# goofoo/SLR

Hardware: AMD Instinct MI355X
Metric: Msamples/sec @1024spp 1280x720 (unidirectional path tracing, Cornell_Box_Spheres-shaped scene) (higher is better)
Workload: dtype f32; 1 GPU; BASELINE configs[1]: Cornell_Box_Spheres walls/light/camera (TestScenes/Cornell_Box_Spheres.txt:8-107,132-138) + two tessellated spheres (aluminium mirror, Lambert), 4428 triangles, RGB mode, 1280x720, 1024 spp, seed 1509761209; stripes=0, tree=host binned SAH

## Files before the change

### include/slrhip.h

```cpp
#ifndef SLRHIP_H
#define SLRHIP_H

#include <stddef.h>
#include <stdint.h>

#ifdef __cplusplus
extern "C" {
#endif

#define SLRHIP_VERSION 7

enum {
    SLRHIP_OK = 0,
    SLRHIP_ERR_INVALID_ARGUMENT = 1,
    SLRHIP_ERR_NO_DEVICE = 2,
    SLRHIP_ERR_HIP = 3,
    SLRHIP_ERR_NO_SCENE = 4,
    SLRHIP_ERR_UNSUPPORTED = 5,
    SLRHIP_ERR_OUT_OF_MEMORY = 6
};

enum {
    SLRHIP_MODE_RGB = 0,
    SLRHIP_MODE_SPECTRAL = 1
// ... 146 lines not shown
    uint64_t shadow_rays;
    uint64_t iterations;
    uint64_t bvh_nodes;
    uint64_t bvh_depth;
    double   build_seconds;
    uint64_t bvh_leaf_references;
} slrhip_counters;

enum {
    SLRHIP_KERNEL_TRACE = 0,
    SLRHIP_KERNEL_SHADE = 1,
    SLRHIP_KERNEL_TAIL = 2,
    SLRHIP_KERNEL_COUNT = 3
};
typedef struct slrhip_profile {
    uint64_t launches[SLRHIP_KERNEL_COUNT];
    double   milliseconds[SLRHIP_KERNEL_COUNT];
    uint64_t rays[2];
    uint64_t nodes[2];
    uint64_t triangles[2];
    uint64_t slot_visits;
} slrhip_profile;

#define SLRHIP_FLAG_DYNAMIC_INSTANCED 1024u
#define SLRHIP_FLAG_DYNAMIC_GEOMETRY 512u
#define SLRHIP_FLAG_NO_PRIMARY_PASS 256u
#define SLRHIP_FLAG_TAIL_KERNEL 128u
#define SLRHIP_FLAG_BVH_SPATIAL_SPLITS 64u
#define SLRHIP_FLAG_BVH_DEVICE_BUILD 4u
#define SLRHIP_FLAG_TEST_DEVICE_ERROR 16u
#define SLRHIP_FLAG_TIME_KERNELS   1u
#define SLRHIP_FLAG_COUNT_TRAVERSAL 2u

typedef struct slrhip_ctx slrhip_ctx;

int slrhip_create(const slrhip_config* config, slrhip_ctx** out_ctx);
int slrhip_destroy(slrhip_ctx* ctx);

int slrhip_upload_scene(slrhip_ctx* ctx, const slrhip_scene_desc* scene);

int slrhip_render_begin(slrhip_ctx* ctx, const slrhip_render_settings* settings, slrhip_shard shard);

int slrhip_render(slrhip_ctx* ctx, uint32_t spp_begin, uint32_t spp_count, void* stream);

int slrhip_resolve_framebuffer(slrhip_ctx* ctx, float* device_dst, size_t num_floats, void* stream);

// ... 308 lines not shown
```

### include/slrhip_debug.h

```cpp
#ifndef SLRHIP_DEBUG_H
#define SLRHIP_DEBUG_H

#include "slrhip.h"

#ifdef __cplusplus
extern "C" {
#endif

int slrhip_bsdf_queries(slrhip_ctx* ctx, uint32_t material, uint32_t n, const float* queries,
                        float wl_offset, float u_lambda, float* out);

int slrhip_debug_work_distribution(uint32_t num_pixels, uint32_t num_slots, uint32_t num_passes, uint32_t run_length,
                                   uint32_t* counts, uint32_t* queue_lengths);

int slrhip_debug_render_plan(int32_t width, int32_t height, uint32_t shard_index, uint32_t shard_count, uint32_t stripes, int32_t mode,
                             uint32_t num_passes, uint64_t budget_bytes, uint32_t* plan, uint32_t* windows, uint32_t max_windows,
                             uint32_t* num_windows, uint32_t* pixels, uint32_t max_pixels);

int slrhip_debug_primary_plan(uint32_t num_pixels, uint32_t num_passes, uint32_t config_flags, int32_t scene_class, uint32_t* plan);

int slrhip_debug_primary_samples(slrhip_ctx* ctx, uint64_t* samples);

int slrhip_debug_primary_entries(uint32_t num_pixels, uint32_t first_pass, uint32_t num_passes, uint32_t window_passes, uint64_t* entries);

int slrhip_debug_primary_stream_plan(uint32_t num_pixels, uint32_t num_passes, uint32_t config_flags, int32_t scene_class, uint64_t* entries);

int slrhip_debug_primary_stream_entries(slrhip_ctx* ctx, uint64_t* entries);

int slrhip_debug_camera_draws(int32_t device, uint32_t n, const uint32_t* tuples, uint32_t* out);

int slrhip_debug_adaptive_blocks(uint32_t spp_min, uint32_t spp_step, uint32_t spp_max, uint32_t* blocks, uint32_t max_blocks,
                                 uint32_t* num_blocks);

int slrhip_debug_modulate_check(const slrhip_modulate_desc* desc);

int slrhip_debug_reproject_check(const slrhip_reproject_desc* desc);

int slrhip_debug_motion_check(int32_t have_render, uint32_t num_instances, const slrhip_motion_desc* desc, uint32_t spp_begin, uint32_t spp_count);

int slrhip_debug_motion_vertices_check(int32_t have_render, uint32_t num_instances, uint32_t config_flags, uint32_t tree_builder,
                                       const slrhip_motion_vertices_desc* desc, uint32_t spp_begin, uint32_t spp_count);

int slrhip_debug_environment_check(const slrhip_environment_desc* desc);

int slrhip_debug_environment(slrhip_ctx* ctx, uint32_t what, float* host_dst, size_t num_floats);

int slrhip_debug_instance_update_check(int32_t have_scene, uint32_t num_instances, const void* device_src, uint32_t first_instance,
                                       uint32_t count);

int slrhip_debug_top_level(slrhip_ctx* ctx, uint32_t what, void* host_dst, size_t num_words);
// ... 43 lines not shown
```

### slr_amd/abi.py

```python
import ctypes as C
import os

import numpy as np

ROOT = os.path.dirname(os.path.dirname(os.path.abspath(__file__)))

MODE_RGB, MODE_SPECTRAL = 0, 1
MAT_MATTE, MAT_METAL, MAT_GLASS, MAT_MF_METAL, MAT_MF_GLASS, MAT_WARD, MAT_ASHIKHMIN, MAT_MULTI = 0, 1, 2, 3, 4, 5, 6, 7
MULTI_INVERSE_0, MULTI_INVERSE_1 = 1, 2
SPEC_RGB_ONLY, SPEC_UPSAMPLED, SPEC_REGULAR, SPEC_IRREGULAR = 0, 1, 2, 3

vertex_dtype = np.dtype([("position", "<f4", 3), ("normal", "<f4", 3), ("tangent", "<f4", 3),
                         ("texcoord", "<f4", 2)])
triangle_dtype = np.dtype([("v", "<u4", 3), ("material", "<u4")])
material_dtype = np.dtype([("type", "<u4"), ("spectrum", "<i4", 3), ("param", "<f4"), ("emittance", "<i4"), ("param2", "<f4"), ("reserved", "<u4")])
spectrum_dtype = np.dtype([("kind", "<u4"), ("rgb", "<f4", 3), ("u", "<f4"), ("v", "<f4"), ("scale", "<f4"),
                           ("lambda_min", "<f4"), ("lambda_max", "<f4"), ("num_samples", "<u4"),
                           ("data_offset", "<u4"), ("reserved", "<u4")])


texture_dtype = np.dtype([("kind", "<u4"), ("offset", "<f4", 2), ("scale", "<f4", 2), ("spectrum", "<i4", 2), ("value", "<f4", 2),
                          ("reserved", "<u4", 3)])
instance_dtype = np.dtype([("first_triangle", "<u4"), ("num_triangles", "<u4"), ("local_to_world", "<f4", 16), ("world_to_local", "<f4", 16)])
instance_transform_dtype = np.dtype([("local_to_world", "<f4", 16), ("world_to_local", "<f4", 16)])
# ... 187 lines not shown
                ("spectra", C.c_void_p), ("num_spectra", C.c_uint32),
                ("spectrum_data", C.c_void_p), ("num_spectrum_data", C.c_uint32),
                ("textures", C.c_void_p), ("num_textures", C.c_uint32),
                ("reserved", C.c_uint32 * 2)]


DENOISE_SIGMA_DISTANCE = 0.1


def noise_metric(summary, metric=NOISE_RMSE):
    if summary["pixels"] == 0:
        return 0.0
    rmse = float(np.sqrt(np.float64(summary["sum_variance_of_mean"]) / np.float64(summary["pixels"])))
    if metric == NOISE_RMSE:
        return rmse
    mean = float(np.float64(summary["sum_mean"]) / np.float64(summary["pixels"]))
    return float("inf") if mean == 0.0 else rmse / mean


FLAG_TIME_KERNELS, FLAG_COUNT_TRAVERSAL, FLAG_BVH_DEVICE_BUILD, FLAG_TEST_DEVICE_ERROR, FLAG_BVH_SPATIAL_SPLITS, FLAG_TAIL_KERNEL = 1, 2, 4, 16, 64, 128
FLAG_NO_PRIMARY_PASS = 256
FLAG_DYNAMIC_GEOMETRY = 512
FLAG_DYNAMIC_INSTANCED = 1024
MAX_STRIPES = 64
KERNEL_NAMES = ("trace", "shade", "tail")

DEFAULT_SEED = 1509761209


class Scene:

    def __init__(self, vertices, triangles, materials, spectra, spectrum_data, camera, env=None, name="scene", textures=None,
                 texture_texels=None, texture_texels_uvs=None, instances=None):
        self.vertices = np.ascontiguousarray(vertices, dtype=vertex_dtype)
        self.triangles = np.ascontiguousarray(triangles, dtype=triangle_dtype)
        mats = np.asarray(materials)
        if mats.dtype != material_dtype:
            conv = np.zeros(len(mats), dtype=material_dtype)
            for name in mats.dtype.names:
                conv[name] = mats[name]
            mats = conv
        self.materials = np.ascontiguousarray(mats, dtype=material_dtype)
        self.spectra = np.ascontiguousarray(spectra, dtype=spectrum_dtype)
        self.spectrum_data = np.ascontiguousarray(spectrum_data, dtype=np.float32)
        self.camera = camera
        self.textures = np.ascontiguousarray(textures if textures is not None else np.zeros(0, texture_dtype), dtype=texture_dtype)
# ... 94 lines not shown
```

### slr_amd/binding.py

```python
import ctypes as C
import os
import subprocess

import numpy as np

from . import abi

CSRC = os.path.join(os.path.dirname(os.path.abspath(__file__)), "csrc")
LIB_PATH = os.path.join(CSRC, "libslrhip.so")

EXPORTS = ["slrhip_create", "slrhip_destroy", "slrhip_upload_scene", "slrhip_render_begin", "slrhip_render",
           "slrhip_resolve_framebuffer", "slrhip_reduce_framebuffer", "slrhip_read_framebuffer", "slrhip_synchronize", "slrhip_get_counters",
           "slrhip_components", "slrhip_get_profile", "slrhip_trace_rays", "slrhip_intersect_rays", "slrhip_test_visibility",
           "slrhip_query_status", "slrhip_render_features", "slrhip_resolve_features", "slrhip_read_features", "slrhip_camera_rays", "slrhip_features_status",
           "slrhip_statistics_begin", "slrhip_resolve_statistics", "slrhip_read_statistics", "slrhip_statistics_summary", "slrhip_render_until", "slrhip_sample_luminance",
           "slrhip_render_adaptive", "slrhip_resolve_framebuffer_mean", "slrhip_read_framebuffer_mean", "slrhip_adaptive_active", "slrhip_debug_adaptive_blocks",
           "slrhip_denoise", "slrhip_denoise_scratch_bytes", "slrhip_tonemap", "slrhip_tonemap_bytes",
           "slrhip_render_albedo", "slrhip_resolve_albedo", "slrhip_read_albedo", "slrhip_modulate", "slrhip_debug_modulate_check",
           "slrhip_clamp_begin", "slrhip_resolve_clamp", "slrhip_read_clamp", "slrhip_clamp_summary", "slrhip_clamp_sample", "slrhip_debug_fold",
           "slrhip_set_environment", "slrhip_env_importance", "slrhip_env_texels_to_uvs", "slrhip_debug_environment_check", "slrhip_debug_environment",
           "slrhip_set_instance_transforms", "slrhip_instances_status", "slrhip_instance_world_box", "slrhip_set_camera",
           "slrhip_debug_instance_update_check", "slrhip_debug_top_level",
           "slrhip_rebuild_top_level", "slrhip_top_level_cost", "slrhip_top_level_key", "slrhip_debug_top_level_rebuild_check",
           "slrhip_debug_top_level_plan", "slrhip_debug_top_level_reseat", "slrhip_debug_top_level_cost", "slrhip_debug_top_level_rebuild",
           "slrhip_render_motion", "slrhip_resolve_motion", "slrhip_read_motion", "slrhip_motion_camera", "slrhip_motion_sample", "slrhip_reproject",
           "slrhip_debug_motion_check", "slrhip_debug_reproject_check",
           "slrhip_render_motion_vertices", "slrhip_motion_sample_vertices", "slrhip_debug_motion_vertices_check",
           "slrhip_debug_tree", "slrhip_debug_host_tree", "slrhip_debug_quantize_nodes",
           "slrhip_set_vertices", "slrhip_geometry_status", "slrhip_debug_geometry_update_check", "slrhip_debug_geometry",
           "slrhip_debug_geometry_update_check2",
           "slrhip_set_materials", "slrhip_set_texture_texels", "slrhip_debug_materials_update_check", "slrhip_debug_materials",
           "slrhip_bsdf_queries", "slrhip_debug_work_distribution", "slrhip_debug_render_plan", "slrhip_debug_primary_plan", "slrhip_debug_primary_samples", "slrhip_debug_primary_entries", "slrhip_debug_primary_stream_entries", "slrhip_debug_primary_stream_plan", "slrhip_debug_camera_draws", "slrhip_sample_seed", "slrhip_upsample", "slrhip_resolve_upsampled", "slrhip_spectrum_to_rgb", "slrhip_tonemap_bgr8", "slrhip_save_bmp",
           "slrhip_last_error_string", "slrhip_version"]


class HipLibraryMissing(RuntimeError):
    pass


class SlrHipError(RuntimeError):
    pass


_lib = None


def build_library():
    subprocess.check_call(["make", "-s", "-C", CSRC])


def load_library():
    global _lib
    if _lib is not None:
        return _lib
    path = os.environ.get("SLRHIP_LIBRARY", LIB_PATH)
# ... 117 lines not shown
                                                                   C.c_uint32]),
                           ("slrhip_debug_geometry", [C.c_void_p, C.c_uint32, C.c_void_p, C.c_size_t])):
        if path == LIB_PATH or hasattr(lib, name):
            getattr(lib, name).argtypes = argtypes
    if path == LIB_PATH or hasattr(lib, "slrhip_debug_geometry_update_check2"):
        lib.slrhip_debug_geometry_update_check2.argtypes = [C.c_int32, C.c_int32, C.c_int32, C.c_uint32, C.c_uint32, C.c_uint32, C.c_void_p, C.c_uint32, C.c_uint32]
    for name, argtypes in (("slrhip_set_materials", [C.c_void_p, C.POINTER(abi.MaterialsDesc), C.c_void_p]),
                           ("slrhip_set_texture_texels", [C.c_void_p, C.c_uint32, C.c_void_p, C.c_uint32, C.c_void_p]),
                           ("slrhip_debug_materials_update_check", [C.c_int32, C.POINTER(abi.SceneDesc), C.c_int32, C.POINTER(abi.MaterialsDesc),
                                                                    C.c_void_p, C.c_size_t]),
                           ("slrhip_debug_materials", [C.c_void_p, C.c_uint32, C.c_void_p, C.c_size_t])):
        if path == LIB_PATH or hasattr(lib, name):
            getattr(lib, name).argtypes = argtypes
    if path == LIB_PATH or hasattr(lib, "slrhip_sample_luminance"):
        lib.slrhip_sample_luminance.restype = C.c_float
    if path == LIB_PATH or hasattr(lib, "slrhip_debug_primary_plan"):
        lib.slrhip_debug_primary_plan.argtypes = [C.c_uint32, C.c_uint32, C.c_uint32, C.c_int32, C.c_void_p]
        lib.slrhip_debug_primary_samples.argtypes = [C.c_void_p, C.POINTER(C.c_uint64)]
    if path == LIB_PATH or hasattr(lib, "slrhip_debug_camera_draws"):
        lib.slrhip_debug_primary_entries.argtypes = [C.c_uint32, C.c_uint32, C.c_uint32, C.c_uint32, C.c_void_p]
        lib.slrhip_debug_primary_stream_entries.argtypes = [C.c_void_p, C.POINTER(C.c_uint64)]
        lib.slrhip_debug_primary_stream_plan.argtypes = [C.c_uint32, C.c_uint32, C.c_uint32, C.c_int32, C.POINTER(C.c_uint64)]
        lib.slrhip_debug_camera_draws.argtypes = [C.c_int32, C.c_uint32, C.c_void_p, C.c_void_p]
    lib.slrhip_bsdf_queries.argtypes = [C.c_void_p, C.c_uint32, C.c_uint32, C.c_void_p, C.c_float, C.c_float, C.c_void_p]
    lib.slrhip_sample_seed.argtypes = [C.c_int32, C.c_uint32, C.c_uint32, C.c_uint32]
    lib.slrhip_sample_seed.restype = C.c_int32
    lib.slrhip_upsample.argtypes = [C.c_int32, C.c_int32, C.c_float, C.c_float, C.c_float, C.c_void_p]
    lib.slrhip_resolve_upsampled.argtypes = [C.POINTER(abi.UpsamplingTables), C.c_float, C.c_float, C.POINTER(C.c_uint32), C.c_void_p]
    lib.slrhip_spectrum_to_rgb.argtypes = [C.c_int32, C.c_void_p, C.c_float, C.c_float, C.c_void_p, C.c_uint32, C.c_void_p]
    lib.slrhip_tonemap_bgr8.argtypes = [C.c_void_p, C.c_int32, C.c_int32, C.c_int32, C.c_float, C.c_void_p, C.c_size_t]
    lib.slrhip_save_bmp.argtypes = [C.c_char_p, C.c_void_p, C.c_int32, C.c_int32]
    lib.slrhip_last_error_string.restype = C.c_char_p
    _lib = lib
    return lib


_hip = None


def _hip_runtime():
    global _hip
    if _hip is None:
        load_library()
        h = C.CDLL("libamdhip64.so.7")
        h.hipMalloc.argtypes = [C.POINTER(C.c_void_p), C.c_size_t]
        h.hipMemcpy.argtypes = [C.c_void_p, C.c_void_p, C.c_size_t, C.c_int]
# ... 286 lines not shown
        return fb

    def _read_plane(self, symbol, channel):
        out = np.empty((self.settings.image_height, self.settings.image_width), np.float32)
        _check(self.lib, getattr(self.lib, symbol)(self.handle, channel, out.ctypes.data, out.size), symbol)
        return out

    def _summary(self, symbol, summary, stream):
        _check(self.lib, getattr(self.lib, symbol)(self.handle, C.byref(summary), self._stream_handle(stream)), symbol)
        return self._summary_dict(summary)

    def synchronize(self):
        _check(self.lib, self.lib.slrhip_synchronize(self.handle), "slrhip_synchronize")

    def counters(self):
        c = abi.Counters()
        _check(self.lib, self.lib.slrhip_get_counters(self.handle, C.byref(c)), "slrhip_get_counters")
        return c

    def primary_samples(self):
        n = C.c_uint64()
        _check(self.lib, self.lib.slrhip_debug_primary_samples(self.handle, C.byref(n)), "slrhip_debug_primary_samples")
        return n.value

    def primary_stream_entries(self):
        n = C.c_uint64()
        _check(self.lib, self.lib.slrhip_debug_primary_stream_entries(self.handle, C.byref(n)), "slrhip_debug_primary_stream_entries")
        return n.value

    def profile(self):
        p = abi.Profile()
        _check(self.lib, self.lib.slrhip_get_profile(self.handle, C.byref(p)), "slrhip_get_profile")
        return p

    def trace_rays(self, org, direction, dist_min, dist_max):
        n = len(org)
        rays = np.zeros((n, 8), np.float32)
        rays[:, 0:3], rays[:, 3:6], rays[:, 6], rays[:, 7] = org, direction, dist_min, dist_max
        hits = np.zeros((n, 4), np.float32)
        _check(self.lib, self.lib.slrhip_trace_rays(self.handle, rays.ctypes.data, n, hits.ctypes.data), "slrhip_trace_rays")
        return hits[:, 0].copy().view(np.uint32), hits[:, 1], hits[:, 2], hits[:, 3]

    def _query(self, rays, stream, outs, call):
        if isinstance(rays, np.ndarray):
            return self._query_host(rays, outs, call)
        import torch
# ... 598 lines not shown
```

### slr_amd/csrc/device_types.h

```cpp
#pragma once
#include <stdint.h>
#include <stdlib.h>

namespace slrhip {

inline const char* tuningEnv(const char* name) {
#ifdef SLR_TUNING_KNOBS
    return getenv(name);
#else
    (void)name;
    return nullptr;
#endif
}

static const uint32_t kInvalidChild = 0xFFFFFFFFu;
static const uint32_t kLeafFlag = 0x80000000u;
static const uint32_t kLeafCountShift = 27;
static const uint32_t kLeafIndexMask = (1u << 27) - 1;
static const uint32_t kMaxLeafTris = 4;
static const uint32_t kPopInstance = 0xFFFFFFFEu;

struct alignas(16) QNode {
    float minx[4], miny[4], minz[4];
    float maxx[4], maxy[4], maxz[4];
    uint32_t child[4];
    uint32_t pad[4];
};
static_assert(sizeof(QNode) == 128, "QNode must be one 128-byte line");

struct alignas(16) QNodeQ {
    float ox, oy, oz, sx;
    float sy, sz; uint32_t qlox, qloy;
    uint32_t qloz, qhix, qhiy, qhiz;
    uint32_t child[4];
};
static_assert(sizeof(QNodeQ) == 64, "QNodeQ must be half a 128-byte line");
// ... 95 lines not shown
```

### slr_amd/csrc/pt_kernels.h

```cpp
#pragma once
#include <hip/hip_runtime.h>
#include <stdint.h>

#include "../../include/slrhip.h"
#include "device_types.h"

namespace slrhip {

static const int kLdsMaterials = 32;
static const int kLdsLights = 16;
static const int kLdsSpectra = 96;
static const int kLdsPoolFloats = 6144;

struct DevScene {
    const float4* nodes;
    const float4* leafTris;
    const ShadeTri* shadeTris;
    const LightTri* lightTris;
    const DevMaterial* materials;
    const DevMaterialS* materialsS;
    const DevSpectrum* spectra;
    const float* spectrumPool;
    const float* lightPMF;
    const float* lightCDF;
// ... 157 lines not shown
    return true;
}

void launchResetSlots(const PathBuffers& pb, const RenderParams& rp, bool clearSensor, hipStream_t stream);
struct ClampParams {
    float4* records;
    float limit;
    uint32_t flags;
};
template <bool kClamp> struct FoldClampArgs {};
template <> struct FoldClampArgs<true> : ClampParams {};
void launchFold(const PathBuffers& pb, const RenderParams& rp, float4* statRecords, const ClampParams& clamp, hipStream_t stream);
void launchShade(const DevScene& sc, const PathBuffers& pb, const RenderParams& rp, uint32_t parity, hipStream_t stream);
void launchCountSamples(const PathBuffers& pb, const RenderParams& rp, hipStream_t stream);
void launchTail(const DevScene& sc, const PathBuffers& pb, const RenderParams& rp, uint32_t liveSlots, int numCUs, hipStream_t stream);
bool tailKernelAvailable(const DevScene& sc, bool spectral);
void launchResolve(const PathBuffers& pb, const RenderParams& rp, float* dst, hipStream_t stream);
void launchBsdfQueries(const DevScene& sc, bool spectral, uint32_t material, uint32_t n, const float* in, float wlOffset, uint32_t wl,
                       float4* geo, float4* misc, float4* fsSample, float4* fsEval, hipStream_t stream);
void launchTraceBatch(const DevScene& sc, const float4* org, const float4* dir, float4* out, uint32_t n, hipStream_t stream);
void launchTraceWs(const DevScene& sc, const PathBuffers& pb, const RenderParams& rp, uint32_t parity, uint32_t blocks, bool count,
                   hipStream_t stream);
int traceWsBlocksPerCU(bool quantizedTree);
void launchPrimary(const DevScene& sc, const PathBuffers& pb, const RenderParams& rp, uint32_t firstPass, uint32_t numPasses, int numCUs,
                   hipStream_t stream);
void launchQueryWs(const DevScene& sc, const float4* rays, uint32_t n, float4* hits, int32_t* instances, uint32_t* visible, uint32_t* errorWord,
                   int numCUs, hipStream_t stream);

struct FeatureParams {
    const uint32_t* pixelXY;
    float4* records;
    float* b2;
    uint32_t* errorWord;
    uint32_t numPixels, numPasses, passBegin;
    uint32_t channels;
    int32_t rngSeed;
    float timeStart, timeEnd;
    uint32_t imageWidth, imageHeight;
};
struct FeatureSums {
    float4* geometric;
    float4* shading;
    float4* tangent;
    uint4* ids;
};
void launchFeatures(const DevScene& sc, const FeatureParams& fp, const FeatureSums& sums, uint32_t idsPass, int numCUs, hipStream_t stream);
void launchCameraRays(const DevScene& sc, const FeatureParams& fp, float4* rays, uint32_t* pixelXY, hipStream_t stream);
void launchCameraDraws(uint32_t n, const uint4* tuples, uint32_t* out, hipStream_t stream);
// ... 62 lines not shown
```

### slr_amd/csrc/pt_trace_indexed.hip

```cpp
#include <hip/hip_runtime.h>

#include "pt_camera.h"
#include "pt_trace_ws.h"

namespace slrhip {

struct WsQueryIO {
    const float4* rays;
    float4* hits;
    int32_t* instances;
    uint32_t* visible;
    uint32_t* error;
    __device__ __forceinline__ uint32_t* errorWord() const { return error; }
    __device__ __forceinline__ uint32_t tag() const { return visible ? kShadowBit : 0u; }
    __device__ __forceinline__ void makeRay(const DevScene&, uint32_t i, float4& o, float4& d) const {
        o = ntLoad4(&rays[2 * (size_t)i]);
        d = ntLoad4(&rays[2 * (size_t)i + 1]);
    }
    __device__ __forceinline__ void produced(uint32_t) const {}
    template <bool INST>
    __device__ __forceinline__ void finish(uint32_t slot, uint32_t hitTri, float hitT, float hitB1, float hitB2, int32_t hitInst) const {
        if (slot & kShadowBit) { visible[slot & ~kShadowBit] = hitTri == 0xFFFFFFFFu ? 1u : 0u; return; }
        const bool miss = hitTri == 0xFFFFFFFFu;
        const float b0 = 1.0f - hitB1 - hitB2;
// ... 84 lines not shown
}

template <bool STREAMS>
static void launchPrimaryWith(const DevScene& sc, const PathBuffers& pb, const RenderParams& rp, uint32_t firstPass, uint32_t numPasses, int numCUs,
                              hipStream_t stream) {
    const uint32_t n = rp.numPixels * numPasses;
    WsPrimaryIO<STREAMS> io{};
    io.stride = rp.spectral ? 4u : 1u;
    io.windowPasses = rp.sppCount;
    const size_t first = windowEntry(0u, firstPass, rp.sppCount);
    io.fp.pixelXY = pb.pixelXY; io.fp.records = pb.results + first * io.stride; io.fp.errorWord = pb.errorWord;
    io.fp.numPixels = rp.numPixels; io.fp.numPasses = numPasses; io.fp.passBegin = rp.sppBegin + firstPass;
    io.fp.rngSeed = rp.rngSeed; io.fp.timeStart = rp.timeStart; io.fp.timeEnd = rp.timeEnd;
    io.fp.imageWidth = rp.imageWidth; io.fp.imageHeight = rp.imageHeight;
    io.instances = pb.primaryInstance ? pb.primaryInstance + first : nullptr;
    io.streams = STREAMS ? pb.primaryRng + first : nullptr;
    io.totals = pb.totals;
    static const int envNc = [] { const char* e = tuningEnv("SLRHIP_PRIMARY_NC"); return e ? atoi(e) : 0; }();
    const int ncTrace = sceneConsumers(sc);
    const int nc = envNc == 3 || envNc == 7 || envNc == 15 ? envNc : (ncTrace == 7 && !sc.instances ? 3 : ncTrace);
    launchRingWs(sc, io, n, nc, numCUs, stream);
}

void launchPrimary(const DevScene& sc, const PathBuffers& pb, const RenderParams& rp, uint32_t firstPass, uint32_t numPasses, int numCUs,
                   hipStream_t stream) {
    const uint32_t n = rp.numPixels * numPasses;
    if (n == 0) return;
    if (pb.primaryRng) launchPrimaryWith<true>(sc, pb, rp, firstPass, numPasses, numCUs, stream);
    else launchPrimaryWith<false>(sc, pb, rp, firstPass, numPasses, numCUs, stream);
}

}
```

### slr_amd/csrc/render_plan.cpp

```cpp
#include "render_plan.h"

#include <algorithm>

#include "../../include/slrhip.h"
#include "pt_kernels.h"

namespace slrhip {

namespace {

uint64_t countCongruent(uint64_t begin, uint64_t end, uint32_t index, uint32_t count) {
    const auto below = [&](uint64_t n) { return n > index ? (n - index + count - 1) / count : 0; };
    return below(end) - below(begin);
}

int refuse(std::string* err, const char* what) {
    *err = std::string("slrhip_render_begin: ") + what;
    return SLRHIP_ERR_INVALID_ARGUMENT;
}

}

int planFrame(int32_t width, int32_t height, uint32_t shardIndex, uint32_t shardCount, uint32_t configStripes, bool spectral,
              long autoStripesOverride, int pairs, FramePlan* out, std::string* err) {
// ... 64 lines not shown

WindowPlan planWindow(uint32_t numPixels, uint32_t sppCount, uint32_t runLengthOverride) {
    WindowPlan w;
    w.workItems = numPixels * sppCount;
    w.runLength = runLengthOverride ? runLengthOverride : kDefaultRunLength;
    while (w.runLength > 1 && (sppCount % w.runLength) != 0) w.runLength /= 2;
    if (sppCount && sppCount % w.runLength) w.runLength = 1;
    w.numRuns = numPixels * (sppCount / std::max(w.runLength, 1u));
    return w;
}

PrimaryPlan planPrimary(uint32_t numPixels, uint32_t sppCount, uint32_t configFlags, bool instanced, bool spectral, bool environment,
                        bool quantized) {
    PrimaryPlan p;
    if ((configFlags & (SLRHIP_FLAG_NO_PRIMARY_PASS | SLRHIP_FLAG_COUNT_TRAVERSAL)) != 0 || numPixels == 0 || sppCount == 0 ||
        numPixels > kPrimaryMaxSamples)
        return p;
    if (spectral || environment) return p;
    p.on = true;
    p.passesPerLaunch = std::min(sppCount, kPrimaryMaxSamples / numPixels);
    p.numLaunches = (sppCount + p.passesPerLaunch - 1) / p.passesPerLaunch;
    p.instanceEntries = instanced ? (uint64_t)numPixels * sppCount : 0u;
    p.rngEntries = instanced || quantized ? 0u : (uint64_t)numPixels * sppCount;
    return p;
}

uint32_t tailSlots(uint32_t numSlots, uint32_t divisor, bool asked, long envTail, bool available) {
    if (!(asked || envTail > 0) || envTail == 0 || !available) return 0u;
    const uint32_t bound = envTail > 0 ? (uint32_t)std::min<long>(envTail, 0x7FFFFFFFL) : kDefaultTailSlots;
    return std::min(bound, numSlots / divisor);
}

uint32_t adaptiveBlock(uint32_t sppMin, uint32_t sppStep, uint32_t sppMax, uint32_t done) {
    if (sppMin < 2 || sppStep == 0 || sppMax < sppMin || done >= sppMax) return 0u;
    return done == 0 ? sppMin : std::min(sppStep, sppMax - done);
}

std::vector<uint32_t> planAdaptiveBlocks(uint32_t sppMin, uint32_t sppStep, uint32_t sppMax) {
    std::vector<uint32_t> blocks;
    for (uint32_t done = 0, n; (n = adaptiveBlock(sppMin, sppStep, sppMax, done)) != 0; done += n) blocks.push_back(n);
    return blocks;
}

DenoiseScratch denoiseScratch(uint32_t width, uint32_t height, uint32_t components) {
    DenoiseScratch s;
    const uint64_t pixels = (uint64_t)width * height;
// ... 218 lines not shown
```

### slr_amd/csrc/render_plan.h

```cpp
#pragma once
#include <stddef.h>
#include <stdint.h>

#include <string>
#include <vector>

#include "../../include/slrhip.h"

namespace slrhip {

const uint32_t kDefaultRunLength = 64;
const uint64_t kFeatureRecordBytes = 512ull << 20;
const uint32_t kDefaultTailSlots = 1u << 18;

struct FramePlan {
    uint32_t width = 0, height = 0;
    uint32_t shardIndex = 0, shardCount = 1;
    bool spectral = false;
    uint32_t numPixels = 0;
    uint32_t stripes = 1;
    uint32_t numSlots = 0;
    size_t slotCapacity = 256;
    uint32_t numBlocks = 1;
    uint32_t shardCapacity = 256;
    uint32_t rayStride = 1, spStride = 1, hdrStride = 1;
};

int planFrame(int32_t width, int32_t height, uint32_t shardIndex, uint32_t shardCount, uint32_t configStripes, bool spectral,
              long autoStripesOverride, int pairs, FramePlan* out, std::string* err);

std::vector<uint32_t> shardPixels(const FramePlan& plan);

uint32_t planWindows(uint32_t numPixels, bool spectral, uint32_t sppCount, uint64_t budgetBytes);

uint32_t featureWindow(uint32_t numPixels, bool wantB2);

struct WindowPlan {
    uint32_t workItems;
    uint32_t runLength;
    uint32_t numRuns;
};
WindowPlan planWindow(uint32_t numPixels, uint32_t sppCount, uint32_t runLengthOverride);

const uint32_t kPrimaryMaxSamples = 0x7FFFFFFFu;
struct PrimaryPlan {
    bool on = false;
    uint32_t passesPerLaunch = 0;
    uint32_t numLaunches = 0;
    uint64_t instanceEntries = 0;
    uint64_t rngEntries = 0;
};
PrimaryPlan planPrimary(uint32_t numPixels, uint32_t sppCount, uint32_t configFlags, bool instanced, bool spectral, bool environment,
                        bool quantized = false);

uint32_t tailSlots(uint32_t numSlots, uint32_t divisor, bool asked, long envTail, bool available);

uint32_t adaptiveBlock(uint32_t sppMin, uint32_t sppStep, uint32_t sppMax, uint32_t done);
std::vector<uint32_t> planAdaptiveBlocks(uint32_t sppMin, uint32_t sppStep, uint32_t sppMax);

struct DenoiseScratch {
    size_t guides = 0, planes[2] = {0, 0}, yv[2] = {0, 0};
    size_t bytes = 0;
};
DenoiseScratch denoiseScratch(uint32_t width, uint32_t height, uint32_t components);

const char* denoiseRefusal(const slrhip_denoise_desc& d);

bool rangesOverlap(const void* a, size_t aBytes, const void* b, size_t bBytes);

// ... 17 lines not shown
```

### slr_amd/csrc/slrhip_api.hip

```cpp
#include <dlfcn.h>

#include <chrono>

#include "pt_refit.h"
#include "slrhip_ctx.h"

using namespace slrhip;

std::atomic<size_t> slrhip::g_skewCounter{0};
static_assert(kClampDropNonFinite == SLRHIP_CLAMP_DROP_NONFINITE, "pt_clamp.h's flag is the ABI's");

const int kDefaultPairs = 1;
#ifndef SLR_TAIL_DIVISOR
#define SLR_TAIL_DIVISOR 8u
#endif

static thread_local std::string g_lastError;

int slrhip::fail(int code, const std::string& msg) {
    g_lastError = msg;
    return code;
}

namespace {
// ... 289 lines not shown
};

int slrhip::renderWindow(slrhip_ctx* ctx, uint32_t sppBegin, uint32_t sppCount, hipStream_t stream, const ActiveWindow* active) {
    RenderParams rp = ctx->params;
    PathBuffers pb = ctx->buffers;
    if (active) { rp.numPixels = active->count; pb.pixelXY = active->xy; }
    const WindowPlan window = planWindow(rp.numPixels, sppCount, runLengthOverride());
    rp.sppBegin = sppBegin; rp.sppCount = sppCount;
    rp.workItems = window.workItems; rp.runLength = window.runLength; rp.numRuns = window.numRuns;
    const PrimaryPlan primary = planPrimary(rp.numPixels, sppCount, ctx->config.flags, ctx->scene.instances != nullptr, rp.spectral != 0,
                                            ctx->scene.hasEnv != 0, ctx->scene.nodesQ != nullptr);
    rp.primary = primary.on ? 1u : 0u;
    pb.primaryInstance = nullptr;
    if (primary.instanceEntries) {
        HIP_TRY(ctx->primaryInstance.alloc((size_t)primary.instanceEntries));
        pb.primaryInstance = ctx->primaryInstance.ptr;
    }
    pb.primaryRng = nullptr;
    if (primary.rngEntries) {
        HIP_TRY(ctx->primaryRng.alloc((size_t)primary.rngEntries));
        pb.primaryRng = ctx->primaryRng.ptr;
    }
    ctx->primaryRngEntries = pb.primaryRng ? ctx->primaryRng.count : 0u;
    launchResetSlots(pb, rp, ctx->firstRenderCall, stream);
    ctx->firstRenderCall = false;
    if (sppCount == 0) return SLRHIP_OK;
    const uint32_t traceBlocks = (uint32_t)ctx->numCUs * (uint32_t)traceWsBlocksPerCU(ctx->scene.nodesQ != nullptr);

    static const long envTail = [] { const char* e = getenv("SLRHIP_TAIL_SLOTS"); return e ? atol(e) : -1L; }();
    const bool counting = (ctx->config.flags & SLRHIP_FLAG_COUNT_TRAVERSAL) != 0;
    rp.tailSlots = tailSlots(rp.numSlots, SLR_TAIL_DIVISOR, (ctx->config.flags & SLRHIP_FLAG_TAIL_KERNEL) != 0 || ctx->config.stripes == 0, envTail,
                             tailKernelAvailable(ctx->scene, rp.spectral != 0) && !counting);

    const bool timeKernels = (ctx->config.flags & SLRHIP_FLAG_TIME_KERNELS) != 0;
    if (timeKernels && ctx->events.empty()) {
        ctx->events.resize((size_t)kCheckEvery * kEventsPerIteration);
        for (hipEvent_t& e : ctx->events) HIP_TRY(hipEventCreate(&e));
    }
    static const char* iterLogPath = getenv("SLRHIP_ITER_LOG");
    std::vector<IterationTimes> iterLog;

    struct PrimaryTimer {
        hipEvent_t t0 = nullptr, t1 = nullptr;
        ~PrimaryTimer() { if (t0) (void)hipEventDestroy(t0); if (t1) (void)hipEventDestroy(t1); }
    } primaryTimer;
    if (primary.on) {
        if (timeKernels) { HIP_TRY(hipEventCreate(&primaryTimer.t0)); HIP_TRY(hipEventCreate(&primaryTimer.t1)); HIP_TRY(hipEventRecord(primaryTimer.t0, stream)); }
        for (uint32_t first = 0; first < sppCount; first += primary.passesPerLaunch)
            launchPrimary(ctx->scene, pb, rp, first, std::min(primary.passesPerLaunch, sppCount - first), ctx->numCUs, stream);
        if (timeKernels) HIP_TRY(hipEventRecord(primaryTimer.t1, stream));
        HIP_TRY(hipGetLastError());
    }

    static const bool noGraph = [] { const char* e = getenv("SLRHIP_GRAPH"); return e && std::string(e) == "0"; }();
    BlockGraph block;
    hipStream_t s = stream;
    if (!timeKernels && !noGraph && rp.numSlots >= (1u << 18)) {
        if (!ctx->workStream) {
            HIP_TRY(hipStreamCreateWithFlags(&ctx->workStream, hipStreamNonBlocking));
            HIP_TRY(hipEventCreateWithFlags(&ctx->userReady, hipEventDisableTiming));
        }
        s = ctx->workStream;
        HIP_TRY(hipEventRecord(ctx->userReady, stream));
        HIP_TRY(hipStreamWaitEvent(s, ctx->userReady, 0));
        HIP_TRY(hipStreamBeginCapture(s, hipStreamCaptureModeThreadLocal));
        (void)launchBlock(ctx, pb, rp, traceBlocks, false, s);
        hipError_t ce = hipStreamEndCapture(s, &block.graph);
        if (ce == hipSuccess) ce = hipGraphInstantiate(&block.exec, block.graph, nullptr, nullptr, 0);
        if (ce != hipSuccess) return fail(SLRHIP_ERR_HIP, std::string("slrhip_render: hipGraph capture failed: ") + hipGetErrorString(ce));
    }

    const uint64_t maxIterations = ((uint64_t)rp.workItems / rp.numSlots + 2) * 128 + 1024;
    uint64_t it = 0;
    uint32_t status[S_TAIL_MODE + 1] = {rp.numSlots, 0u, 0u, 0u};
// ... 326 lines not shown
```

### slr_amd/csrc/slrhip_ctx.h

```cpp
#pragma once
#include <hip/hip_runtime.h>

#include <algorithm>
#include <atomic>
#include <cstdio>
#include <cstring>
#include <string>
#include <vector>

#include "../../include/slrhip.h"
#include "bvh.h"
#include "materials_prep.h"
#include "pt_clamp.h"
#include "pt_kernels.h"
#include "pt_motion.h"
#include "render_plan.h"
#include "scene_prep.h"

namespace slrhip {

const uint32_t kStatusWords = 8;
enum StatusWord : uint32_t {
    S_LIVE = 0, S_ERROR = 1,
    S_TAIL_IDLED = 2, S_TAIL_MODE = 3,
// ... 104 lines not shown
    bool envOwnMap = false;
    DevArray<uint8_t> gridCells;
    DevArray<float> pointUV, pointSpectrum;
    slrhip::DevScene scene;
    uint32_t bvhDepth = 0;
    uint64_t bvhLeafRefs = 0;
    uint32_t treeBuilder = 0;
    double buildSeconds = 0.0;

    slrhip_render_settings settings;
    slrhip_shard shard;
    slrhip::RenderParams params;
    DevArray<uint32_t> pixelXY;
    DevArray<uint4> rng;
    DevArray<float4> rayOrg, rayDir, hit, alpha, spR, spC, nee, shadowDir;
    DevArray<float4> results, fbSum, fbComp;
    DevArray<uint32_t> cursor, idleShards;
    DevArray<float> pdfPrev;
    DevArray<uint4> hdr;
    DevArray<int32_t> hitInstance;
    DevArray<int32_t> primaryInstance;
    DevArray<uint4> primaryRng;
    uint64_t primaryRngEntries = 0;
    DevArray<uint32_t> flags, visible, shadowQueue, tailList, queueCount, activeSlots, blockDead;
    DevArray<uint64_t> totals;
    DevArray<float> resolveScratch;
    DevArray<uint32_t> queryError;
    DevArray<float4> featGeometric, featShading, featTangent, featRecords;
    DevArray<float> featB2;
    DevArray<uint4> featIds;
    DevArray<uint32_t> featError;
    uint32_t featChannels = 0;
    uint32_t featWindow = 0;
    uint64_t featPassEnd = 0;
    bool featErrorReady = false;
    DevArray<float> albSums;
    bool albReady = false;
    uint32_t albWindow = 0;
    uint64_t albPasses = 0;
    DevArray<float4> motionSums;
    bool motionReady = false;
    uint32_t motionWindow = 0;
    uint32_t motionVerticesWindow = 0;
    slrhip::PixelRecords<slrhip::StatsTotals> stats;
    slrhip::PixelRecords<slrhip::ClampTotals> clamp;
    float clampLimit = 0.0f;
// ... 61 lines not shown
```

### slr_amd/csrc/slrhip_diagnostics.hip

```cpp
#include <memory>

#include "../../include/slrhip_debug.h"
#include "slrhip_ctx.h"

using namespace slrhip;

static void hitsToUV(float* hits, uint32_t n) {
    for (uint32_t i = 0; i < n; ++i) {
        float* h = hits + (size_t)i * 4;
        const float b1 = h[2], b2 = h[3];
        const float b0 = 1.0f - b1 - b2;
        uint32_t tri; std::memcpy(&tri, h, 4);
        h[2] = tri == 0xFFFFFFFFu ? 0.0f : b0;
        h[3] = tri == 0xFFFFFFFFu ? 0.0f : b1;
    }
}

extern "C" {

int slrhip_trace_rays(slrhip_ctx* ctx, const float* rays, uint32_t n, float* hits) {
    if (!ctx || !rays || !hits) return fail(SLRHIP_ERR_INVALID_ARGUMENT, "slrhip_trace_rays: null argument");
    if (!ctx->haveScene) return fail(SLRHIP_ERR_NO_SCENE, "slrhip_trace_rays: no scene uploaded");
    if (n == 0) return SLRHIP_OK;
    HIP_TRY(hipSetDevice(ctx->device));
// ... 137 lines not shown
}

int slrhip_debug_primary_entries(uint32_t numPixels, uint32_t firstPass, uint32_t numPasses, uint32_t windowPasses, uint64_t* entries) {
    if (!entries) return fail(SLRHIP_ERR_INVALID_ARGUMENT, "slrhip_debug_primary_entries: null argument");
    if (numPasses == 0 || (uint64_t)firstPass + numPasses > windowPasses || (uint64_t)numPixels * numPasses > kPrimaryMaxSamples)
        return fail(SLRHIP_ERR_INVALID_ARGUMENT, "slrhip_debug_primary_entries: the launch's passes must be 1 or more, inside the window, and under 2^31 samples");
    const size_t first = windowEntry(0u, firstPass, windowPasses);
    for (uint32_t i = 0; i < numPixels * numPasses; ++i) entries[i] = first + primaryLaunchEntry(i, numPasses, windowPasses);
    return SLRHIP_OK;
}

int slrhip_debug_primary_stream_plan(uint32_t numPixels, uint32_t numPasses, uint32_t configFlags, int32_t sceneClass, uint64_t* entries) {
    if (!entries) return fail(SLRHIP_ERR_INVALID_ARGUMENT, "slrhip_debug_primary_stream_plan: null argument");
    *entries = planPrimary(numPixels, numPasses, configFlags, (sceneClass & 1) != 0, (sceneClass & 2) != 0, (sceneClass & 4) != 0, (sceneClass & 8) != 0).rngEntries;
    return SLRHIP_OK;
}

int slrhip_debug_primary_stream_entries(slrhip_ctx* ctx, uint64_t* entries) {
    if (!ctx || !entries) return fail(SLRHIP_ERR_INVALID_ARGUMENT, "slrhip_debug_primary_stream_entries: null argument");
    *entries = ctx->primaryRngEntries;
    return SLRHIP_OK;
}

int slrhip_debug_camera_draws(int32_t device, uint32_t n, const uint32_t* tuples, uint32_t* out) {
    if (!tuples || !out) return fail(SLRHIP_ERR_INVALID_ARGUMENT, "slrhip_debug_camera_draws: null argument");
    if (n == 0) return SLRHIP_OK;
    HIP_TRY(hipSetDevice(device));
    DevArray<uint4> dIn;
    DevArray<uint32_t> dOut;
    HIP_TRY(dIn.alloc(n));
    HIP_TRY(dOut.alloc((size_t)n * 16u));
    HIP_TRY(hipMemcpy(dIn.ptr, tuples, (size_t)n * sizeof(uint4), hipMemcpyHostToDevice));
    launchCameraDraws(n, dIn.ptr, dOut.ptr, nullptr);
    HIP_TRY(hipGetLastError());
    HIP_TRY(hipDeviceSynchronize());
    HIP_TRY(hipMemcpy(out, dOut.ptr, (size_t)n * 16u * sizeof(uint32_t), hipMemcpyDeviceToHost));
    return SLRHIP_OK;
}

}

namespace {
const uint32_t kTreeSummaryWords = 16, kTreeArrays = 7;
struct TreeView {
    uint32_t summary[kTreeSummaryWords];
    const void* src[kTreeArrays];
// ... 128 lines not shown
```

Before: 3255 Msamples/s.

## Add direct one-thread-per-sample primary ray kernel replacing ring work-stealing for primaries

Adds a new primary-ray kernel that assigns each camera sample to its own thread. Each thread generates the camera ray, traverses the float BVH with an LDS stack, and writes the hit record and RNG state directly with non-temporal stores. This replaces the ring/work-stealing primary kernel by default when RNG streams are used (no instancing or quantized tree), removing queue management overhead for coherent primary rays. The old path stays available behind a new PRIMARY_RING flag, and debug entry points are added. The risk is load imbalance, since there is no stealing.

Measured after the change: 3435 Msamples/s (median of 6 runs). 1.06x the previous value.

```diff
diff --git a/include/slrhip.h b/include/slrhip.h
--- a/include/slrhip.h
+++ b/include/slrhip.h
@@ -192,6 +192,7 @@
     uint64_t slot_visits;
 } slrhip_profile;
 
+#define SLRHIP_FLAG_PRIMARY_RING 2048u
 #define SLRHIP_FLAG_DYNAMIC_INSTANCED 1024u
 #define SLRHIP_FLAG_DYNAMIC_GEOMETRY 512u
 #define SLRHIP_FLAG_NO_PRIMARY_PASS 256u
diff --git a/include/slrhip_debug.h b/include/slrhip_debug.h
--- a/include/slrhip_debug.h
+++ b/include/slrhip_debug.h
@@ -26,6 +26,13 @@
 int slrhip_debug_primary_stream_plan(uint32_t num_pixels, uint32_t num_passes, uint32_t config_flags, int32_t scene_class, uint64_t* entries);
 
 int slrhip_debug_primary_stream_entries(slrhip_ctx* ctx, uint64_t* entries);
+
+int slrhip_debug_primary_kernel_plan(uint32_t num_pixels, uint32_t num_passes, uint32_t config_flags, int32_t scene_class, uint32_t* direct);
+
+int slrhip_debug_primary_kernel(slrhip_ctx* ctx, uint32_t* kernel);
+
+int slrhip_debug_primary_pass(slrhip_ctx* ctx, uint32_t kernel, uint32_t first_pass, uint32_t num_passes, uint32_t window_passes, void* records,
+                              void* streams);
 
 int slrhip_debug_camera_draws(int32_t device, uint32_t n, const uint32_t* tuples, uint32_t* out);
 
diff --git a/slr_amd/abi.py b/slr_amd/abi.py
--- a/slr_amd/abi.py
+++ b/slr_amd/abi.py
@@ -233,6 +233,7 @@
 FLAG_NO_PRIMARY_PASS = 256
 FLAG_DYNAMIC_GEOMETRY = 512
 FLAG_DYNAMIC_INSTANCED = 1024
+FLAG_PRIMARY_RING = 2048
 MAX_STRIPES = 64
 KERNEL_NAMES = ("trace", "shade", "tail")
 
diff --git a/slr_amd/binding.py b/slr_amd/binding.py
--- a/slr_amd/binding.py
+++ b/slr_amd/binding.py
@@ -30,7 +30,7 @@
            "slrhip_set_vertices", "slrhip_geometry_status", "slrhip_debug_geometry_update_check", "slrhip_debug_geometry",
            "slrhip_debug_geometry_update_check2",
            "slrhip_set_materials", "slrhip_set_texture_texels", "slrhip_debug_materials_update_check", "slrhip_debug_materials",
-           "slrhip_bsdf_queries", "slrhip_debug_work_distribution", "slrhip_debug_render_plan", "slrhip_debug_primary_plan", "slrhip_debug_primary_samples", "slrhip_debug_primary_entries", "slrhip_debug_primary_stream_entries", "slrhip_debug_primary_stream_plan", "slrhip_debug_camera_draws", "slrhip_sample_seed", "slrhip_upsample", "slrhip_resolve_upsampled", "slrhip_spectrum_to_rgb", "slrhip_tonemap_bgr8", "slrhip_save_bmp",
+           "slrhip_bsdf_queries", "slrhip_debug_work_distribution", "slrhip_debug_render_plan", "slrhip_debug_primary_plan", "slrhip_debug_primary_samples", "slrhip_debug_primary_entries", "slrhip_debug_primary_stream_entries", "slrhip_debug_primary_stream_plan", "slrhip_debug_primary_kernel_plan", "slrhip_debug_primary_kernel", "slrhip_debug_primary_pass", "slrhip_debug_camera_draws", "slrhip_sample_seed", "slrhip_upsample", "slrhip_resolve_upsampled", "slrhip_spectrum_to_rgb", "slrhip_tonemap_bgr8", "slrhip_save_bmp",
            "slrhip_last_error_string", "slrhip_version"]
 
 
@@ -194,6 +194,10 @@
         lib.slrhip_debug_primary_stream_entries.argtypes = [C.c_void_p, C.POINTER(C.c_uint64)]
         lib.slrhip_debug_primary_stream_plan.argtypes = [C.c_uint32, C.c_uint32, C.c_uint32, C.c_int32, C.POINTER(C.c_uint64)]
         lib.slrhip_debug_camera_draws.argtypes = [C.c_int32, C.c_uint32, C.c_void_p, C.c_void_p]
+    if path == LIB_PATH or hasattr(lib, "slrhip_debug_primary_pass"):
+        lib.slrhip_debug_primary_kernel_plan.argtypes = [C.c_uint32, C.c_uint32, C.c_uint32, C.c_int32, C.POINTER(C.c_uint32)]
+        lib.slrhip_debug_primary_kernel.argtypes = [C.c_void_p, C.POINTER(C.c_uint32)]
+        lib.slrhip_debug_primary_pass.argtypes = [C.c_void_p, C.c_uint32, C.c_uint32, C.c_uint32, C.c_uint32, C.c_void_p, C.c_void_p]
     lib.slrhip_bsdf_queries.argtypes = [C.c_void_p, C.c_uint32, C.c_uint32, C.c_void_p, C.c_float, C.c_float, C.c_void_p]
     lib.slrhip_sample_seed.argtypes = [C.c_int32, C.c_uint32, C.c_uint32, C.c_uint32]
     lib.slrhip_sample_seed.restype = C.c_int32
@@ -526,6 +530,15 @@
         n = C.c_uint64()
         _check(self.lib, self.lib.slrhip_debug_primary_samples(self.handle, C.byref(n)), "slrhip_debug_primary_samples")
         return n.value
+
+    def primary_kernel(self):
+        k = C.c_uint32(0)
+        _check(self.lib, self.lib.slrhip_debug_primary_kernel(self.handle, C.byref(k)), "slrhip_debug_primary_kernel")
+        return int(k.value)
+
+    def primary_pass(self, kernel, first_pass, num_passes, window_passes, records, streams=0):
+        _check(self.lib, self.lib.slrhip_debug_primary_pass(self.handle, kernel, first_pass, num_passes, window_passes, records, streams or None),
+               "slrhip_debug_primary_pass")
 
     def primary_stream_entries(self):
         n = C.c_uint64()
diff --git a/slr_amd/csrc/device_types.h b/slr_amd/csrc/device_types.h
--- a/slr_amd/csrc/device_types.h
+++ b/slr_amd/csrc/device_types.h
@@ -12,6 +12,8 @@
     return nullptr;
 #endif
 }
+
+enum class PrimaryKernel : uint32_t { None = 0, Ring = 1, Direct = 2 };
 
 static const uint32_t kInvalidChild = 0xFFFFFFFFu;
 static const uint32_t kLeafFlag = 0x80000000u;
diff --git a/slr_amd/csrc/pt_kernels.h b/slr_amd/csrc/pt_kernels.h
--- a/slr_amd/csrc/pt_kernels.h
+++ b/slr_amd/csrc/pt_kernels.h
@@ -203,8 +203,10 @@
 void launchTraceWs(const DevScene& sc, const PathBuffers& pb, const RenderParams& rp, uint32_t parity, uint32_t blocks, bool count,
                    hipStream_t stream);
 int traceWsBlocksPerCU(bool quantizedTree);
-void launchPrimary(const DevScene& sc, const PathBuffers& pb, const RenderParams& rp, uint32_t firstPass, uint32_t numPasses, int numCUs,
-                   hipStream_t stream);
+void launchPrimary(const DevScene& sc, const PathBuffers& pb, const RenderParams& rp, uint32_t firstPass, uint32_t numPasses, PrimaryKernel kernel,
+                   int numCUs, hipStream_t stream);
+void launchPrimaryDirect(const DevScene& sc, const PathBuffers& pb, const RenderParams& rp, uint32_t firstPass, uint32_t numPasses, float4* records,
+                         uint4* streams, int numCUs, hipStream_t stream);
 void launchQueryWs(const DevScene& sc, const float4* rays, uint32_t n, float4* hits, int32_t* instances, uint32_t* visible, uint32_t* errorWord,
                    int numCUs, hipStream_t stream);
 
diff --git a/slr_amd/csrc/pt_primary_direct.hip b/slr_amd/csrc/pt_primary_direct.hip
--- /dev/null
+++ b/slr_amd/csrc/pt_primary_direct.hip
@@ -0,0 +1,89 @@
+#include <hip/hip_runtime.h>
+
+#include <algorithm>
+#include <string>
+
+#include "pt_camera.h"
+#include "pt_trace_ws.h"
+#include "pt_traverse.h"
+
+namespace slrhip {
+
+struct PrimaryDirectIO {
+    FeatureParams fp;
+    uint4* streams;
+    uint64_t* totals;
+    uint32_t stride;
+    uint32_t windowPasses;
+};
+
+struct PrimaryDirectLds {
+    uint32_t stack[kLdsStack * kTraceBlock];
+};
+
+template <bool STREAMS, bool PERSISTENT, bool WAVE_PIXEL>
+__global__ __launch_bounds__(kTraceBlock) __attribute__((amdgpu_waves_per_eu(8, 8)))
+void k_primary_direct(DevScene sc, PrimaryDirectIO io, uint32_t n) {
+    __shared__ PrimaryDirectLds lds;
+    uint32_t rays = 0;
+    for (uint32_t base = blockIdx.x * kTraceBlock; base < n; base += gridDim.x * kTraceBlock) {
+        rays += min(n - base, (uint32_t)kTraceBlock);
+        const uint32_t i = base + threadIdx.x;
+        if (i < n) {
+            float4 o, d;
+            size_t entry;
+            {
+                const uint32_t pix = WAVE_PIXEL ? (uint32_t)__builtin_amdgcn_readfirstlane((int)(i / io.fp.numPasses)) : i / io.fp.numPasses;
+                const uint32_t pass = i - pix * io.fp.numPasses;
+                uint32_t xy;
+                Rng after;
+                cameraRayOf(sc.camera, io.fp, pix, pass, o, d, xy, after);
+                entry = (size_t)i + (size_t)pix * (io.windowPasses - io.fp.numPasses);
+                if constexpr (STREAMS)
+                    ntStore4(reinterpret_cast<float4*>(io.streams + entry),
+                             make_float4(__uint_as_float(after.s0), __uint_as_float(after.s1), __uint_as_float(after.s2), __uint_as_float(after.s3)));
+            }
+            HitRec hit;
+            TravCount cnt;
+            traverse<false, false, false>(sc, sc.nodes, sc.leafTris, nullptr, 0u, V3(o.x, o.y, o.z), V3(d.x, d.y, d.z), o.w, d.w, &hit,
+                                          lds.stack + threadIdx.x, &cnt, io.fp.errorWord);
+            ntStore4(io.fp.records + entry * io.stride, make_float4(__uint_as_float(hit.tri), hit.t, hit.b1, hit.b2));
+        }
+        if (!PERSISTENT) break;
+    }
+    if (threadIdx.x == 0 && rays) atomicAdd((unsigned long long*)&io.totals[totalIndex(T_EXT_RAYS, blockIdx.x % kShards)], (unsigned long long)rays);
+}
+
+void launchPrimaryDirect(const DevScene& sc, const PathBuffers& pb, const RenderParams& rp, uint32_t firstPass, uint32_t numPasses, float4* records,
+                         uint4* streams, int numCUs, hipStream_t stream) {
+    const uint32_t n = rp.numPixels * numPasses;
+    if (n == 0) return;
+    PrimaryDirectIO io{};
+    io.stride = rp.spectral ? 4u : 1u;
+    io.windowPasses = rp.sppCount;
+    io.fp.pixelXY = pb.pixelXY; io.fp.records = records; io.fp.errorWord = pb.errorWord;
+    io.fp.numPixels = rp.numPixels; io.fp.numPasses = numPasses; io.fp.passBegin = rp.sppBegin + firstPass;
+    io.fp.rngSeed = rp.rngSeed; io.fp.timeStart = rp.timeStart; io.fp.timeEnd = rp.timeEnd;
+    io.fp.imageWidth = rp.imageWidth; io.fp.imageHeight = rp.imageHeight;
+    io.streams = streams;
+    io.totals = pb.totals;
+    const dim3 grid((n + kTraceBlock - 1) / kTraceBlock), block(kTraceBlock);
+#ifdef SLR_TUNING_KNOBS
+    static const std::string variant = [] { const char* e = tuningEnv("SLRHIP_PRIMARY_DIRECT"); return std::string(e ? e : ""); }();
+    if (variant == "persistent") {
+        const dim3 resident(std::min((uint32_t)numCUs * 8u, grid.x));
+        if (streams) hipLaunchKernelGGL((k_primary_direct<true, true, false>), resident, block, 0, stream, sc, io, n);
+        else hipLaunchKernelGGL((k_primary_direct<false, true, false>), resident, block, 0, stream, sc, io, n);
+        return;
+    }
+    if (variant == "wavepixel" && numPasses % 64u == 0u) {
+        if (streams) hipLaunchKernelGGL((k_primary_direct<true, false, true>), grid, block, 0, stream, sc, io, n);
+        else hipLaunchKernelGGL((k_primary_direct<false, false, true>), grid, block, 0, stream, sc, io, n);
+        return;
+    }
+#endif
+    if (streams) hipLaunchKernelGGL((k_primary_direct<true, false, false>), grid, block, 0, stream, sc, io, n);
+    else hipLaunchKernelGGL((k_primary_direct<false, false, false>), grid, block, 0, stream, sc, io, n);
+}
+
+}
diff --git a/slr_amd/csrc/pt_trace_indexed.hip b/slr_amd/csrc/pt_trace_indexed.hip
--- a/slr_amd/csrc/pt_trace_indexed.hip
+++ b/slr_amd/csrc/pt_trace_indexed.hip
@@ -130,10 +130,16 @@
     launchRingWs(sc, io, n, nc, numCUs, stream);
 }
 
-void launchPrimary(const DevScene& sc, const PathBuffers& pb, const RenderParams& rp, uint32_t firstPass, uint32_t numPasses, int numCUs,
-                   hipStream_t stream) {
+void launchPrimary(const DevScene& sc, const PathBuffers& pb, const RenderParams& rp, uint32_t firstPass, uint32_t numPasses, PrimaryKernel kernel,
+                   int numCUs, hipStream_t stream) {
     const uint32_t n = rp.numPixels * numPasses;
     if (n == 0) return;
+    if (kernel == PrimaryKernel::Direct) {
+        const size_t first = windowEntry(0u, firstPass, rp.sppCount);
+        launchPrimaryDirect(sc, pb, rp, firstPass, numPasses, pb.results + first * (rp.spectral ? 4u : 1u), pb.primaryRng ? pb.primaryRng + first : nullptr,
+                            numCUs, stream);
+        return;
+    }
     if (pb.primaryRng) launchPrimaryWith<true>(sc, pb, rp, firstPass, numPasses, numCUs, stream);
     else launchPrimaryWith<false>(sc, pb, rp, firstPass, numPasses, numCUs, stream);
 }
diff --git a/slr_amd/csrc/render_plan.cpp b/slr_amd/csrc/render_plan.cpp
--- a/slr_amd/csrc/render_plan.cpp
+++ b/slr_amd/csrc/render_plan.cpp
@@ -110,6 +110,7 @@
     p.numLaunches = (sppCount + p.passesPerLaunch - 1) / p.passesPerLaunch;
     p.instanceEntries = instanced ? (uint64_t)numPixels * sppCount : 0u;
     p.rngEntries = instanced || quantized ? 0u : (uint64_t)numPixels * sppCount;
+    p.kernel = p.rngEntries && !(configFlags & SLRHIP_FLAG_PRIMARY_RING) ? PrimaryKernel::Direct : PrimaryKernel::Ring;
     return p;
 }
 
diff --git a/slr_amd/csrc/render_plan.h b/slr_amd/csrc/render_plan.h
--- a/slr_amd/csrc/render_plan.h
+++ b/slr_amd/csrc/render_plan.h
@@ -6,6 +6,7 @@
 #include <vector>
 
 #include "../../include/slrhip.h"
+#include "device_types.h"
 
 namespace slrhip {
 
@@ -45,6 +46,7 @@
 const uint32_t kPrimaryMaxSamples = 0x7FFFFFFFu;
 struct PrimaryPlan {
     bool on = false;
+    PrimaryKernel kernel = PrimaryKernel::None;
     uint32_t passesPerLaunch = 0;
     uint32_t numLaunches = 0;
     uint64_t instanceEntries = 0;
diff --git a/slr_amd/csrc/slrhip_api.hip b/slr_amd/csrc/slrhip_api.hip
--- a/slr_amd/csrc/slrhip_api.hip
+++ b/slr_amd/csrc/slrhip_api.hip
@@ -335,6 +335,7 @@
         pb.primaryRng = ctx->primaryRng.ptr;
     }
     ctx->primaryRngEntries = pb.primaryRng ? ctx->primaryRng.count : 0u;
+    ctx->primaryKernel = PrimaryKernel::None;
     launchResetSlots(pb, rp, ctx->firstRenderCall, stream);
     ctx->firstRenderCall = false;
     if (sppCount == 0) return SLRHIP_OK;
@@ -360,9 +361,10 @@
     if (primary.on) {
         if (timeKernels) { HIP_TRY(hipEventCreate(&primaryTimer.t0)); HIP_TRY(hipEventCreate(&primaryTimer.t1)); HIP_TRY(hipEventRecord(primaryTimer.t0, stream)); }
         for (uint32_t first = 0; first < sppCount; first += primary.passesPerLaunch)
-            launchPrimary(ctx->scene, pb, rp, first, std::min(primary.passesPerLaunch, sppCount - first), ctx->numCUs, stream);
+            launchPrimary(ctx->scene, pb, rp, first, std::min(primary.passesPerLaunch, sppCount - first), primary.kernel, ctx->numCUs, stream);
         if (timeKernels) HIP_TRY(hipEventRecord(primaryTimer.t1, stream));
         HIP_TRY(hipGetLastError());
+        ctx->primaryKernel = primary.kernel;
     }
 
     static const bool noGraph = [] { const char* e = getenv("SLRHIP_GRAPH"); return e && std::string(e) == "0"; }();
diff --git a/slr_amd/csrc/slrhip_ctx.h b/slr_amd/csrc/slrhip_ctx.h
--- a/slr_amd/csrc/slrhip_ctx.h
+++ b/slr_amd/csrc/slrhip_ctx.h
@@ -150,6 +150,7 @@
     DevArray<int32_t> primaryInstance;
     DevArray<uint4> primaryRng;
     uint64_t primaryRngEntries = 0;
+    slrhip::PrimaryKernel primaryKernel = slrhip::PrimaryKernel::None;
     DevArray<uint32_t> flags, visible, shadowQueue, tailList, queueCount, activeSlots, blockDead;
     DevArray<uint64_t> totals;
     DevArray<float> resolveScratch;
diff --git a/slr_amd/csrc/slrhip_diagnostics.hip b/slr_amd/csrc/slrhip_diagnostics.hip
--- a/slr_amd/csrc/slrhip_diagnostics.hip
+++ b/slr_amd/csrc/slrhip_diagnostics.hip
@@ -183,6 +183,54 @@
     return SLRHIP_OK;
 }
 
+int slrhip_debug_primary_kernel_plan(uint32_t numPixels, uint32_t numPasses, uint32_t configFlags, int32_t sceneClass, uint32_t* direct) {
+    if (!direct) return fail(SLRHIP_ERR_INVALID_ARGUMENT, "slrhip_debug_primary_kernel_plan: null argument");
+    *direct = planPrimary(numPixels, numPasses, configFlags, (sceneClass & 1) != 0, (sceneClass & 2) != 0, (sceneClass & 4) != 0, (sceneClass & 8) != 0).kernel ==
+                      PrimaryKernel::Direct
+                  ? 1u
+                  : 0u;
+    return SLRHIP_OK;
+}
+
+int slrhip_debug_primary_kernel(slrhip_ctx* ctx, uint32_t* kernel) {
+    if (!ctx || !kernel) return fail(SLRHIP_ERR_INVALID_ARGUMENT, "slrhip_debug_primary_kernel: null argument");
+    *kernel = (uint32_t)ctx->primaryKernel;
+    return SLRHIP_OK;
+}
+
+int slrhip_debug_primary_pass(slrhip_ctx* ctx, uint32_t kernel, uint32_t firstPass, uint32_t numPasses, uint32_t windowPasses, void* records,
+                              void* streams) {
+    if (!ctx || !records) return fail(SLRHIP_ERR_INVALID_ARGUMENT, "slrhip_debug_primary_pass: null argument");
+    if (!ctx->haveRender) return fail(SLRHIP_ERR_NO_SCENE, "slrhip_debug_primary_pass: call slrhip_render_begin first");
+    if (kernel > 1u) return fail(SLRHIP_ERR_INVALID_ARGUMENT, "slrhip_debug_primary_pass: kernel is 0 (ring) or 1 (direct)");
+    RenderParams rp = ctx->params;
+    PathBuffers pb = ctx->buffers;
+    if (numPasses == 0 || (uint64_t)firstPass + numPasses > windowPasses || (uint64_t)rp.numPixels * numPasses > kPrimaryMaxSamples ||
+        (uint64_t)rp.numPixels * windowPasses > 0xFFFFFFFFull)
+        return fail(SLRHIP_ERR_INVALID_ARGUMENT, "slrhip_debug_primary_pass: the launch's passes must be 1 or more, inside the window, and under 2^31 samples");
+    if (kernel == 1u && (ctx->scene.instances || ctx->scene.nodesQ))
+        return fail(SLRHIP_ERR_UNSUPPORTED, "slrhip_debug_primary_pass: the direct kernel traces scenes without instances on the float nodes only");
+    if (rp.numSlots == 0) return SLRHIP_OK;
+    HIP_TRY(hipSetDevice(ctx->device));
+    HIP_TRY(hipDeviceSynchronize());
+    rp.sppBegin = 0; rp.sppCount = windowPasses;
+    pb.results = static_cast<float4*>(records);
+    pb.primaryRng = static_cast<uint4*>(streams);
+    pb.primaryInstance = nullptr;
+    if (ctx->scene.instances) {
+        HIP_TRY(ctx->primaryInstance.alloc((size_t)rp.numPixels * windowPasses));
+        pb.primaryInstance = ctx->primaryInstance.ptr;
+    }
+    HIP_TRY(hipMemset(pb.errorWord, 0, sizeof(uint32_t)));
+    launchPrimary(ctx->scene, pb, rp, firstPass, numPasses, kernel ? PrimaryKernel::Direct : PrimaryKernel::Ring, ctx->numCUs, nullptr);
+    HIP_TRY(hipGetLastError());
+    HIP_TRY(hipDeviceSynchronize());
+    uint32_t bits = 0;
+    HIP_TRY(hipMemcpy(&bits, pb.errorWord, sizeof(bits), hipMemcpyDeviceToHost));
+    if (bits) return fail(SLRHIP_ERR_HIP, "slrhip_debug_primary_pass: device-side error word set: " + std::to_string(bits));
+    return SLRHIP_OK;
+}
+
 int slrhip_debug_camera_draws(int32_t device, uint32_t n, const uint32_t* tuples, uint32_t* out) {
     if (!tuples || !out) return fail(SLRHIP_ERR_INVALID_ARGUMENT, "slrhip_debug_camera_draws: null argument");
     if (n == 0) return SLRHIP_OK;
```
